# facebookresearch/NeRF-Det

Hardware: AMD Instinct MI355X
Metric: scenes/sec (50-view 240x320, 40x40x16 voxels) (higher is better)
Workload: dtype f32 (convolutions: fp32 operands as hi + lo fp16 pairs of the power-of-two pre-scaled tensors, three products per multiply on the fp16 MFMA, fp32 accumulate; error against fp64 at or below the six-product bf16x3 form's; a device-side range guard repeats a scene on bf16x3 when part of a tensor falls ; 1 GPU; cfg2: nerfdet_res50_2x_low_res forward_test, 50 views 240x320, 40x40x16 voxels, fp32, 1 scene/step/GPU, random-init weights; parallelism=scene replicas x1 (no data-path collective)

## Files before the change

include/nerfdet_hip.h:

```cpp
#ifndef NERFDET_HIP_H
#define NERFDET_HIP_H

#include <stdint.h>

#ifdef __cplusplus
extern "C" {
#endif

#define NDET_OK 0
#define NDET_E_INVALID (-1)
#define NDET_E_UNSUPPORTED (-2)
#define NDET_E_LAUNCH (-3)

#define NDET_LAYOUT_CN 0
#define NDET_LAYOUT_NC 1

int ndet_version(void);
const char* ndet_last_error(void);

int ndet_get_points(float* points, int nx, int ny, int nz, const float* voxel_size_host,
                    const float* origin_host, void* stream);

int ndet_nchw_to_nhwc(const float* src, float* dst, int n, int c, int hw, void* stream);

// ... 264 lines not shown
                      const float* residual, int relu, int splits, int tile, void* workspace, void* stream);

int ndet_conv_ndhwc(const float* in, const float* w_packed, float* out, int D, int H, int W, int Cin, int Cout,
                    const int* kernel_host, const int* stride_host, const int* pad_host, const float* scale,
                    const float* shift, const float* residual, int residual_up2, int relu, int splits, int tile,
                    void* workspace, void* stream);

int ndet_split_weights_bf16x3(const float* w_packed, int taps, int Cout, int Cin, uint16_t* planes, void* stream);

int ndet_split_weights_bf16x3_torch(const float* w_torch, int taps, int Cout, int Cin, int adjoint, uint16_t* planes, void* stream);

int ndet_point_mlp_alpha(const float* points, const float* global_feat, int N, int F, int K0, int hidden, const uint16_t* const* w_planes_host,
                         const float* w_inv_scale_host, const float* const* bias_host, const float* w_sigma, const float* b_sigma,
                         float* raw_sigma, float* alpha, float* h_out, void* stream);

int ndet_split_weights_f16x2(const float* w_packed, int taps, int Cout, int Cin, float scale, uint16_t* planes, void* stream);

int ndet_amax_f32(const float* x, int64_t n, float* slot, void* stream);

int ndet_amax_slot_floats(void);

int ndet_measurement_knob(const char* name_host, int64_t value);

typedef struct NdetConvArgs {
    int32_t size;
    const float* in;
    const uint16_t* w_planes;
    float* out;
    int D, H, W, Cin, Cout;
    int kernel[3], stride[3], pad[3];
    int transposed;
    const float* scale;
    const float* shift;
    const float* residual;
    int residual_up2, relu, splits, tile, arith;
    const float* in_amax;
    float w_inv_scale;
    const float* w_amax;
    float* out_amax;
    void* workspace;
    unsigned* guard;
    float guard_l1, guard_tol;
    int keep_partials;
    const float* map_w;
    const float* map_b;
    float* map_out;
} NdetConvArgs;
int ndet_conv_split(const NdetConvArgs* a, void* stream);

int ndet_conv_split_batch(const NdetConvArgs* a, int batch, void* stream);

int ndet_conv_halo_patch(int tile, int D, int H, int W, const int* kernel, int* patch, int* looped);

#define NDET_TILE_DIRECT 1
#define NDET_TILE_OWNS_ROWS 2
#define NDET_TILE_ORDER2 4
int ndet_conv_tile_info(int tile, int* rows, int* cols, int* flags);

int ndet_conv_chain(const float* in, const uint16_t* w_planes, int D, int H, int W, int Cin, int Cmid, const int* kernel,
                    const int* stride, const int* pad, const float* scale1, const float* shift1, const uint16_t* w3_planes,
                    int Cout, const float* scale3, const float* shift3, const float* residual, int relu3, float* out,
                    int arith, const float* in_amax, float w1_inv_scale, float w3_inv_scale, float* out_amax, float guard_l1,
                    float guard_l1_3, float guard_tol, unsigned* guard, void* stream);

int ndet_bottleneck_f16x2(const float* x, int N, int H, int W, int Cin, int Cout, const uint16_t* w1_planes, float w1_inv_scale, const float* scale1,
                          const float* shift1, const uint16_t* w2_planes, float w2_inv_scale, const float* scale2, const float* shift2,
                          const uint16_t* w3_planes, float w3_inv_scale, const float* scale3, const float* shift3, const uint16_t* wd_planes,
                          float wd_inv_scale, const float* scale_d, const float* shift_d, const float* in_amax, float* out_amax, float* out,
                          const float* guard_l1_host, float guard_tol, unsigned* guard, void* stream);

int ndet_bn_relu_maxpool_nhwc(const float* x, const float* scale, const float* shift, int N, int H, int W, int C,
                              float* out, void* stream);

int ndet_stem_pack_weights(const float* w_64x3x7x7, uint16_t* planes , void* stream);
int ndet_stem_pack_weights_f16x2(const float* w_64x3x7x7, float scale, uint16_t* planes , void* stream);

int ndet_stem_conv_bn_relu_maxpool(const float* images, int N, int H, int W, int64_t stride_n, int64_t stride_c, int64_t stride_y,
                                   int64_t stride_x, const uint16_t* w_planes, float w_inv_scale, const float* scale, const float* shift, float* out, float* out_amax,
                                   void* stream);

int ndet_normalize_views(const uint8_t* frames_bgr, const int* ids, int n_sel, int H, int W, const double* mean_rgb,
                         const double* std_rgb, float* img, float* denorm, void* stream);

int ndet_target_rays(const uint8_t* frames_bgr, const int* target_ids, int n_targets, int H, int W, int margin,
                     const float* intrinsic_rows, const float* camrotc2w, const float* cam_lightpos, const double* mean_rgb,
                     const double* std_rgb, float* raydirs, float* lightpos, float* gt_images, void* stream);

int ndet_resize_normalize_views(const uint8_t* frames_bgr, const int* ids, int n_sel, int Hs, int Ws, int Hr, int Wr, int H, int W,
                                const double* mean_rgb, const double* std_rgb, float* img, float* denorm, uint8_t* resized_bgr,
                                void* stream);

int ndet_resize_normalize_views_nv12(const uint8_t* surfaces, const int* ids, int n_sel, int Hs, int Ws, int pitch, int uv_row, int rows,
                                     int Hr, int Wr, int H, int W, const double* mean_rgb, const double* std_rgb, float* img, float* denorm,
                                     uint8_t* resized_bgr, void* stream);

int ndet_nv12_to_bgr(const uint8_t* surfaces, const int* ids, int n_sel, int Hs, int Ws, int pitch, int uv_row, int rows,
                     uint8_t* frames_bgr, void* stream);

int ndet_bgr_to_nv12(const uint8_t* frames_bgr, int n, int H, int W, uint8_t* surfaces, void* stream);

int ndet_depth_frames(const uint16_t* frames_mm, const int* ids, int n_sel, int Hd, int Wd, int h, int w, int margin, double* out,
                      void* stream);

int ndet_positive_indices(const double* x, int64_t n, int64_t* indices, int64_t* count, void* workspace, void* stream);

int ndet_camera_rays(const float* intrinsic_rows, const float* camrotc2w, const float* cam_lightpos, int n_cams, int x0, int y0, int stride,
// ... 84 lines not shown
```

nerf-det_amd/_lib.py:

```python
from __future__ import annotations

import ctypes
import os
from ctypes import c_char_p, c_float, c_int, c_int64, c_void_p

_HERE = os.path.dirname(os.path.abspath(__file__))
LIB_PATH = os.path.join(_HERE, "lib", "libnerfdet_hip.so")

NDET_LAYOUT_CN = 0
NDET_LAYOUT_NC = 1

_P = c_void_p
_F3 = ctypes.POINTER(c_float)


class NdetConvArgs(ctypes.Structure):
    _fields_ = ([("size", ctypes.c_int32), ("in_", _P), ("w_planes", _P), ("out", _P)] + [(f, c_int) for f in ("D", "H", "W", "Cin", "Cout")]
                + [(f, c_int * 3) for f in ("kernel", "stride", "pad")] + [("transposed", c_int), ("scale", _P), ("shift", _P), ("residual", _P)]
                + [(f, c_int) for f in ("residual_up2", "relu", "splits", "tile", "arith")] + [("in_amax", _P), ("w_inv_scale", c_float)]
                + [(f, _P) for f in ("w_amax", "out_amax", "workspace", "guard")] + [("guard_l1", c_float), ("guard_tol", c_float), ("keep_partials", c_int)]
                + [(f, _P) for f in ("map_w", "map_b", "map_out")])


class NdetDepthGate(ctypes.Structure):
# ... 74 lines not shown
                               _P, _P, _P, _G, _P], c_int),
    "ndet_scene_density_finish": ([_S, _P, _P, _P], c_int),
    "ndet_scene_volume_finish": ([_S, _P, _P, _P, _P], c_int),
    "ndet_scene_density_finish_ring": ([_S, c_int, _P, _P, _P], c_int),
    "ndet_scene_volume_finish_ring": ([_S, c_int, _P, _P, _P, _P], c_int),
    "ndet_scene_group_check": ([_SG, _GS, c_int], c_int),
    "ndet_scene_accumulate_group": ([_SG, _GS, c_int, _P, c_int, c_int, c_int64, c_int64, _P, c_int64, c_int64, _P, _P, c_int, c_int, c_int64, c_int64,
                                     c_int64, _P, _P, _G, _P], c_int),
    "ndet_scene_density_finish_group": ([_SG, _GS, _P, _P, _P], c_int),
    "ndet_scene_volume_finish_group": ([_SG, _GS, _P, _P, _P, _P], c_int),
    "ndet_scene_group_ring_check": ([_SG, _GR, _P], c_int),
    "ndet_scene_density_finish_group_ring": ([_SG, _GR, _P, _P, _P, _P, _P], c_int),
    "ndet_scene_volume_finish_group_ring": ([_SG, _GR, _P, _P, _P, _P, _P, _P], c_int),
    "ndet_alpha_gate": ([_P, _P, _P, _P, c_int, c_int, c_int, _P], c_int),
    "ndet_sigma_to_alpha": ([_P, _P, c_int, _P], c_int),
    "ndet_posenc_concat": ([_P, _P, c_int, c_int, c_int, _P, _P], c_int),
    "ndet_sigma_head": ([_P, c_int, _P, c_int, c_int, _P, _P, c_int, _P, _P, _P], c_int),
    "ndet_nms_workspace_bytes": ([c_int], c_int64),
    "ndet_aligned_3d_nms": ([_P, _P, _P, c_int, c_float, _P, _P, _P, _P], c_int),
    "ndet_head_decode": ([_P, c_int, _P, _P, c_int, c_int, c_int, _F3, _F3, _P, _P, _P, _P], c_int),
    "ndet_head_decode_levels": ([c_int, _P, _P, _P, _P, _P, _P, c_int, _P, c_int, c_int, c_int, _P, _P, _P, _P], c_int),
    "ndet_sample_along_rays": ([_P, _P, c_int, c_int, c_float, c_float, _P, _P, _P, _P], c_int),
    "ndet_ray_view_stats": ([_P, c_int, _P, c_int, c_float, c_float, _P, c_int, c_int, c_int64, c_int64, c_int64,
                             _P, c_int, c_int, c_int, c_int64, c_int64, _P, _P, _P, _P], c_int),
    "ndet_pack_rgb_nhwc4": ([_P, c_int, c_int, c_int, c_int64, c_int64, c_int64, _P, _P], c_int),
    "ndet_ray_view_stats_packed": ([_P, c_int, _P, c_int, c_float, c_float, _P, c_int, c_int, _P, c_int, c_int, c_int, c_int64, c_int64,
                                    _P, _P, _P, _P], c_int),
    "ndet_ray_view_stats_bank": ([_P, c_int, _P, c_int, c_float, c_float, c_int, c_int, c_int, c_int, c_int, _P, _P, _P, _P], c_int),
    "ndet_ray_view_stats_bank_group": ([_P, ctypes.POINTER(NdetBankGroupSel), c_float, c_float, c_int, c_int, c_int, c_int, c_int, _P, _P, _P, _P], c_int),
    "ndet_occupancy_bits": ([_P, _P, c_int, c_int, c_int, c_float, c_int, _P, _P], c_int),
    "ndet_cull_blocks": ([c_int64], c_int64),
    "ndet_cull_count": ([_P, c_int64, _P, ctypes.POINTER(c_int), _F3, _F3, c_int, _P, _P], c_int),
    "ndet_cull_write": ([_P, c_int64, _P, ctypes.POINTER(c_int), _F3, _F3, c_int, _P, _P, _P, _P], c_int),
    "ndet_ray_view_count_bank": ([_P, c_int64, _P, c_int, c_float, c_float, _P, _P, _P], c_int),
    "ndet_ray_advance": ([_P, _P, c_int, c_int, c_int, c_int, _P], c_int),
    "ndet_front_blocks": ([c_int64, c_int], c_int64),
    "ndet_front_count": ([_P, c_int, c_int, c_int, c_int, _P, c_float, _P, ctypes.POINTER(c_int), _F3, _F3, c_int, _P, _P], c_int),
    "ndet_front_write": ([_P, c_int, c_int, c_int, c_int, _P, c_float, _P, ctypes.POINTER(c_int), _F3, _F3, c_int, _P, _P, _P, _P], c_int),
    "ndet_ray_view_stats_packed_bwd": ([_P, _P, c_int, _P, c_int, c_float, c_float, _P, c_int, c_int, c_int, c_int64, c_int64, _P, _P], c_int),
    "ndet_project_sample": ([_P, c_int, _P, c_int, c_float, c_float, _P, c_int, c_int, c_int64, c_int64, c_int64,
                             _P, c_int, c_int, c_int, c_int64, c_int64, _P, _P, _P], c_int),
    "ndet_composite": ([_P, _P, _P, c_int, c_int, c_int, _P, _P, _P, _P, _P, _P, _P, _P], c_int),
    "ndet_sample_pdf": ([_P, _P, c_int, c_int, _P, c_int, c_int, _P, _P], c_int),
    "ndet_importance_merge": ([_P, _P, _P, _P, c_int, c_int, _P, c_int, c_int, _P, _P, _P, _P], c_int),
    "ndet_backproject_aggregate_bwd": ([_P, c_int, c_int, c_int, c_int, c_int, c_int64, c_int64, _P, c_int, _P, _P, _P], c_int),
    "ndet_density_features_bwd": ([_P, _P, c_int, c_int, c_int, c_int, c_int64, c_int64, _P, _P, c_int, _P, _P, _P, _P], c_int),
    "ndet_ray_view_stats_bwd": ([_P, _P, c_int, _P, c_int, c_float, c_float, _P, c_int, c_int, c_int, c_int64, c_int64, _P, _P], c_int),
    "ndet_composite_bwd": ([_P, _P, _P, c_int, c_int, c_int, _P, _P, _P, _P, _P], c_int),
    "ndet_split_weights_bf16x3": ([_P, c_int, c_int, c_int, _P, _P], c_int),
    "ndet_split_weights_f16x2": ([_P, c_int, c_int, c_int, c_float, _P, _P], c_int),
    "ndet_conv_split": ([ctypes.POINTER(NdetConvArgs), _P], c_int),
    "ndet_conv_split_batch": ([ctypes.POINTER(NdetConvArgs), c_int, _P], c_int),
    "ndet_conv_halo_patch": ([c_int] * 4 + [ctypes.POINTER(c_int)] * 3, c_int),
    "ndet_conv_tile_info": ([c_int] + [ctypes.POINTER(c_int)] * 3, c_int),
    "ndet_conv_chain": ([_P, _P] + [c_int] * 5 + [_P] * 6 + [c_int, _P, _P, _P, c_int, _P, c_int, _P, c_float, c_float, _P, c_float, c_float, c_float, _P, _P], c_int),
    "ndet_bottleneck_f16x2": ([_P, c_int, c_int, c_int, c_int, c_int, _P, c_float, _P, _P, _P, c_float, _P, _P, _P, c_float, _P, _P, _P, c_float, _P, _P, _P, _P, _P,
                               _P, c_float, _P, _P], c_int),
    "ndet_amax_f32": ([_P, ctypes.c_int64, _P, _P], c_int),
    "ndet_amax_slot_floats": ([], c_int),
    "ndet_point_mlp_alpha": ([_P, _P, c_int, c_int, c_int, c_int, _P, _P, _P, _P, _P, _P, _P, _P, _P], c_int),
    "ndet_measurement_knob": ([c_char_p, c_int64], c_int),
    "ndet_split_weights_bf16x3_torch": ([_P, c_int, c_int, c_int, c_int, _P, _P], c_int),
    "ndet_level_valid": ([_P, c_int, c_int, c_int, c_int, _P, _P], c_int),
    "ndet_select_candidates": ([c_int, _P, _P, _P, _P, c_float, _P, _P, _P, _P, _P], c_int),
    "ndet_select_candidates_topk": ([c_int, _P, _P, _P, _P, c_float, c_int, _P, _P, _P, _P, _P], c_int),
    "ndet_gather_detections": ([_P, c_int, _P, _P, _P, _P, _P, _P, _P], c_int),
    "ndet_nms_pack_detections": ([_P, _P, _P, _P, c_int, c_int, c_int, c_float, _P, _P, _P, _P, c_int, _P, _P], c_int),
    "ndet_normalize_views": ([_P, _P, c_int, c_int, c_int, _P, _P, _P, _P, _P], c_int),
    "ndet_target_rays": ([_P, _P, c_int, c_int, c_int, c_int, _P, _P, _P, _P, _P, _P, _P, _P, _P], c_int),
    "ndet_resize_normalize_views": ([_P, _P] + [c_int] * 7 + [_P] * 6, c_int),
    "ndet_resize_normalize_views_nv12": ([_P, _P] + [c_int] * 10 + [_P] * 6, c_int),
    "ndet_nv12_to_bgr": ([_P, _P] + [c_int] * 6 + [_P, _P], c_int),
    "ndet_bgr_to_nv12": ([_P] + [c_int] * 3 + [_P, _P], c_int),
    "ndet_depth_frames": ([_P, _P] + [c_int] * 6 + [_P, _P], c_int),
    "ndet_positive_indices": ([_P, c_int64, _P, _P, _P, _P], c_int),
    "ndet_positive_indices_workspace_bytes": ([c_int64], c_int64),
    "ndet_camera_rays": ([_P, _P, _P] + [c_int] * 6 + [_P, _P, _P], c_int),
    "ndet_pack_frames": ([_P, _P, _P, c_int64, _P, _P, _P], c_int),
    "ndet_frame_errors": ([_P, _P, _P, _P, c_int, c_int64, _P, _P], c_int),
    "ndet_frame_ssim": ([_P, _P, _P, c_int, c_int, c_int, c_int, _P, _P], c_int),
    "ndet_project_boxes": ([_P, _P, _P] + [c_int] * 7 + [c_float, _P, _P, _P, _P, _P], c_int),
    "ndet_draw_boxes": ([_P, _P, _P, _P] + [c_int] * 5 + [_P, _P], c_int),
    "ndet_label_frames": ([_P] * 5 + [c_int] * 7 + [_P, _P], c_int),
    "ndet_stem_pack_weights": ([_P, _P, _P], c_int),
    "ndet_stem_conv_bn_relu_maxpool": ([_P, c_int, c_int, c_int, c_int64, c_int64, c_int64, c_int64, _P, c_float, _P, _P, _P, _P, _P], c_int),
    "ndet_stem_pack_weights_f16x2": ([_P, c_float, _P, _P], c_int),
    "ndet_wgrad_dy_planes": ([_P, c_int, c_int, c_int, _P, _P], c_int),
    "ndet_wgrad_dy_planes_f16x2": ([_P, c_int, c_int, c_int, _P, _P, _P], c_int),
    "ndet_bn_workspace_floats": ([c_int64, c_int], c_int64),
    "ndet_bn_train_forward": ([_P, c_int64, c_int, _P, _P, _P, _P, c_float, c_float, _P, c_int, _P, _P, _P, _P, _P, _P], c_int),
    "ndet_bn_train_backward": ([_P, _P, _P, c_int64, c_int, _P, _P, _P, c_int, _P, _P, _P, _P, _P, _P, _P], c_int),
    "ndet_wgrad_to_torch": ([_P, c_int, c_int, c_int, c_int, _P, _P], c_int),
    "ndet_split_weights_train": ([_P, c_int, c_int, c_int, c_int, _P, _P, _P, _P], c_int),
    "ndet_relu_affine_bwd": ([_P, _P, _P, c_int64, c_int, c_int, _P, _P, _P], c_int),
    "ndet_relu_affine_bwd_amax": ([_P, _P, _P, c_int64, c_int, c_int, _P, _P, _P, _P], c_int),
    "ndet_wgrad_split": ([_P] + [c_int] * 4 + [_P, _P, _P, _P] + [c_int] * 4 + [_P, _P, _P, _P, c_int, _P], c_int),
    "ndet_wgrad_rows": ([_P] + [c_int] * 4 + [_P, _P, _P] + [c_int] * 3 + [_P, _P], c_int),
    "ndet_bn_relu_maxpool_nhwc": ([_P, _P, _P, c_int, c_int, c_int, c_int, _P, _P], c_int),
    "ndet_conv3d_workspace_bytes": ([c_int] * 8, c_int64),
    "ndet_conv_ndhwc": ([_P, _P, _P, c_int, c_int, c_int, c_int, c_int, ctypes.POINTER(c_int), ctypes.POINTER(c_int),
                         ctypes.POINTER(c_int), _P, _P, _P, c_int, c_int, c_int, c_int, _P, _P], c_int),
    "ndet_conv3d_ndhwc": ([_P, _P, _P, c_int, c_int, c_int, c_int, c_int, c_int, c_int, c_int, _P, _P, _P, c_int, c_int, c_int,
                           _P, _P], c_int),
}

_lib = None
# ... 58 lines not shown
```

nerf-det_amd/csrc/conv_split_kernels.hip:

```cpp
#include "conv_common.hpp"

#include "spl_common.hpp"

#include <type_traits>

template <int BM, int BN, int WGM, int WGN, int SCH, bool BATCH = false>
__device__ __forceinline__ void conv_split_mainloop(const Conv3dParams& p, const uint16_t* __restrict__ wsplit, uint16_t* lds16,
                                                    f32x16 (&acc)[BM / WGM / 32][BN / WGN / 32], int& ztap) {
    constexpr int NTHR = 64 * WGM * WGN;
    constexpr int WM = BM / WGM, WN = BN / WGN;
    constexpr int MT = WM / 32, NT = WN / 32;
    constexpr int RPA = NTHR / 8;
    constexpr int RPB = NTHR / 4;
    constexpr int AR = BM / RPA, BR = BN / RPB;
    static_assert(AR >= 1 && BR >= 1 && MT >= 1 && NT >= 1, "tile too small for the thread count");
    constexpr int APL = BM * SPL_RS, BPL = BN * SPL_RS;
    constexpr int NPL = Spl<SCH>::NPL, WPL = Spl<SCH>::WPL;
    const float xs = SCH == 1 ? conv_xscale(p.amax_in) : 1.0f;
    uint16_t* As = lds16;
    uint16_t* Bs = lds16 + NPL * APL;

    const int tid = threadIdx.x;
    const int lane = tid & 63, wave = tid >> 6;
    const int wm = wave / WGN, wn = wave % WGN;
// ... 1188 lines not shown
    NDET_REQUIRE(taps <= 32, NDET_E_UNSUPPORTED, "%s: the persistent 128x256 tile supports at most 32 taps", fn);
    NDET_REQUIRE(p.Cout % 16 == 0, NDET_E_UNSUPPORTED, "%s: the persistent 128x256 tile needs Cout %% 16 == 0", fn);
    NDET_REQUIRE((int64_t)p.D * p.H * p.W * p.Cin * 4 < ((int64_t)1 << 31) && (int64_t)taps * p.Cin * p.Cout * 6 < ((int64_t)1 << 31) &&
                     ((int64_t)p.M + 128) * p.Cout * 4 < ((int64_t)1 << 31),
                 NDET_E_UNSUPPORTED, "%s: the persistent 128x256 tile addresses at most 2 GB per operand", fn);
    const int n_mt = (p.M + BM - 1) / BM, n_nt = (p.Cout + WS_BN - 1) / WS_BN;
    const int64_t n_tiles = (int64_t)n_mt * n_nt * p.splits;
    static int n_cu = 0;
    if (n_cu == 0) {
        int dev = 0;
        hipDeviceProp_t prop;
        if (hipGetDevice(&dev) != hipSuccess || hipGetDeviceProperties(&prop, dev) != hipSuccess) n_cu = 256;
        else n_cu = prop.multiProcessorCount > 0 ? prop.multiProcessorCount : 256;
    }
    const int grid = (int)(n_tiles < n_cu ? n_tiles : n_cu);
    const int sch = conv_scheme(p);
    const size_t lds = (size_t)2 * (sch == 2 ? 1 : (sch == 1 ? 2 : 3)) * (BM + WS_BN) * CBK * sizeof(uint16_t);
    return with_scheme(sch, [&](auto s) -> int {
        const auto kernel = k_conv_split_wsp<decltype(s)::value, BM, NCONS>;
        NDET_RAISE_LDS(kernel, lds);
        hipLaunchKernelGGL(kernel, dim3(grid), dim3(64 * (NCONS + 4)), lds, st, p, (const uint16_t*)p.w, n_mt, n_nt);
        return NDET_OK;
    });
}


struct HaloGeom {
    int ltd, lth, ltw;
    int npd, nph, npw;
    int HH, HW, NH;
    int T;
    int KDL;
    int Tin;
};

struct HaloRowMap {
    int first, ltw, lth, d0, h0, w0, OD, OH, OW;
    __device__ __forceinline__ int operator()(int row) const {
        const int r = first + row;
        const int tw = r & ((1 << ltw) - 1), th = (r >> ltw) & ((1 << lth) - 1), td = r >> (ltw + lth);
        const int od = d0 + td, oh = h0 + th, ow = w0 + tw;
        return (od < OD && oh < OH && ow < OW) ? (od * OH + oh) * OW + ow : -1;
    }
};
struct HaloRowMapBatch {
    HaloRowMap in_volume;
    int vol_first;
    __device__ __forceinline__ int operator()(int row) const {
        const int m = in_volume(row);
        return m < 0 ? m : vol_first + m;
    }
};

template <int NT16, int WGN, int SCHB, int NPROD = 4>
__global__ __launch_bounds__(64 * (2 * WGN + NPROD), 1) void k_conv_split_halo(const Conv3dParams p, const uint16_t* __restrict__ wsplit, const HaloGeom g) {
    constexpr int SCH = SCHB & 3;
    constexpr bool BATCH = (SCHB & SPL_BATCH) != 0;
    constexpr int BN = 16 * NT16 * WGN;
    constexpr int NCONS = 2 * WGN, NTHR = 64 * (NCONS + NPROD);
    constexpr int PT = 64 * NPROD;
    constexpr int HALO_MAX = (BN == 128) ? 400 : 224;
    constexpr int NSTAGE = (BN == 128) ? 3 : 2;
    constexpr int NPIECE = (HALO_MAX * 8 + PT - 1) / PT;
    constexpr int APL = HALO_MAX * CBK, BPL = BN * CBK;
    constexpr int NPL = SCH == 1 ? 2 : (SCH == 2 ? 1 : 3);
    constexpr int WPL = SCH == 1 ? 2 : 3;
    constexpr int BSTAGE = NPL * BPL;
    constexpr int BR = BN / (16 * NPROD);
    static_assert(BR >= 1 && BN % (16 * NPROD) == 0, "every producer wave stages 16 rows of each row group");
    constexpr int NB = NPL * BR;
    extern __shared__ __attribute__((aligned(16))) uint16_t lds16[];
    uint16_t* Bs = lds16 + NPL * APL;

    const int tid = threadIdx.x;
    const int lane = tid & 63;
    const int wave = __builtin_amdgcn_readfirstlane(tid >> 6);
    const bool consumer = wave < NCONS;
    const int wm = (wave % NCONS) / WGN, wn = (wave % NCONS) % WGN;
    const ConvBlock blk = conv_block(p);
    const int n0 = blk.y * BN;
    const int TH = 1 << g.lth, TW = 1 << g.ltw;
    int pb = blk.x;
    const int pwi = pb % g.npw; pb /= g.npw;
    const int phi = pb % g.nph;
    const int pdv = pb / g.nph;
    const int vol = BATCH ? pdv / g.npd : 0;
    const int pdi = BATCH ? pdv - vol * g.npd : pdv;
    const int d0 = pdi << g.ltd, h0 = phi << g.lth, w0 = pwi << g.ltw;
    const float amax_in = conv_amax_in(p);
    conv_guard_check(p, amax_in);

    const int nch_all = p.Cin / CBK;
    int cb = 0, ce = nch_all;
    if (p.splits > 1) {
        cb = (int)((int64_t)nch_all * blk.z / p.splits);
        ce = (int)((int64_t)nch_all * (blk.z + 1) / p.splits);
    }
    const int nch = ce - cb;
    const int T = g.T, Tin = g.Tin;
    const int S = nch * T;
    const int nphase = nch * g.KDL;

    f32x4v acc[4][NT16];
#pragma unroll
    for (int a = 0; a < 4; ++a)
#pragma unroll
        for (int b = 0; b < NT16; ++b) acc[a][b] = (f32x4v){0.f, 0.f, 0.f, 0.f};

    if (!consumer) {
        const int stid = tid - 64 * NCONS;
        const int pw4 = wave - NCONS;
        const float xs = SCH == 1 ? conv_xscale(p.amax_in) : 1.0f;
        const int64_t slice = (int64_t)p.H * p.W * p.Cin;
        const bool dloop = g.KDL > 1;
        const __amdgpu_buffer_rsrc_t ares = __builtin_amdgcn_make_buffer_rsrc((void*)(p.in - (dloop ? p.pd * slice : 0)), 0, WS_OOB, 0x00020000);
        const __amdgpu_buffer_rsrc_t bres = __builtin_amdgcn_make_buffer_rsrc((void*)wsplit, 0, WS_OOB, 0x00020000);
        unsigned avoff[NPIECE], adst[NPIECE], amask[NPIECE];
#pragma unroll
        for (int i = 0; i < NPIECE; ++i) {
            const int idx = stid + PT * i;
            const int row = idx >> 3, q = idx & 7;
            const int hw = row % g.HW, hh = (row / g.HW) % g.HH, hd = row / (g.HW * g.HH);
            const int vd = d0 + hd - (dloop ? 0 : p.pd), vh = h0 - p.ph + hh, vw = w0 - p.pw + hw;
            const bool ok = row < g.NH && (unsigned)vd < (unsigned)p.D && (unsigned)vh < (unsigned)p.H && (unsigned)vw < (unsigned)p.W;
            if constexpr (BATCH) avoff[i] = ok ? (unsigned)((((int64_t)(vol * p.D + vd) * p.H + vh) * p.W + vw) * p.Cin * 4 + q * 16) : WS_OOB;
            else avoff[i] = ok ? (unsigned)((((int64_t)vd * p.H + vh) * p.W + vw) * p.Cin * 4 + q * 16) : WS_OOB;
            unsigned msk = 0;
            if (dloop)
                for (int k = 0; k < g.KDL; ++k)
                    if ((unsigned)(vd + k - p.pd) >= (unsigned)p.D) msk |= 1u << k;
            amask[i] = msk;
            adst[i] = row < g.NH ? (unsigned)((row * CBK + (((q >> 1) ^ ws_swz(row)) * 8) + (q & 1) * 4) * 2) : ~0u;
        }
        unsigned bvoff[BR];
#pragma unroll
        for (int i = 0; i < BR; ++i) {
            const int row = (stid >> 2) + (PT / 4) * i, co = n0 + row;
            bvoff[i] = co < p.Cout ? (unsigned)((co * CBK + (((stid & 3) ^ ws_swz(row)) * 8)) * 2) : WS_OOB;
        }
        const unsigned wtile_b = (unsigned)p.Cout * CBK * 2;
        int dt = 0, dc = 0;
        auto dma_b = [&](int u) {
            const unsigned soff = __builtin_amdgcn_readfirstlane((unsigned)(((int64_t)dt * nch_all + cb + dc) * WPL) * wtile_b);
            uint16_t* stage = Bs + (u % NSTAGE) * BSTAGE;
#pragma unroll
            for (int i = 0; i < BR; ++i)
#pragma unroll
                for (int pl = 0; pl < NPL; ++pl) {
                    uint16_t* dst = stage + pl * BPL + ((PT / 4) * i + pw4 * 16) * CBK;
                    spl_dma16(bres, dst, bvoff[i], __builtin_amdgcn_readfirstlane(soff + pl * wtile_b));
                }
            if (++dt == T) { dt = 0; ++dc; }
        };
        u32x4 ra[NPIECE];
        auto load_a = [&](int a) {
            const int c = a / g.KDL, kdl = a - c * g.KDL;
            const unsigned soff = __builtin_amdgcn_readfirstlane((unsigned)(((cb + c) * CBK + (dloop ? kdl * slice : 0)) * 4));
            const unsigned sh = 31 - kdl;
#pragma unroll
            for (int i = 0; i < NPIECE; ++i) ra[i] = __builtin_amdgcn_raw_buffer_load_b128(ares, ((amask[i] << sh) & WS_OOB) | avoff[i], soff, 0);
        };
        auto split_store_a = [&]() {
            char* base = reinterpret_cast<char*>(lds16);
#pragma unroll
            for (int i = 0; i < NPIECE; ++i) {
                const u32x4 u = ra[i];
                uint2 s0, s1, s2;
                const float4 xv = make_float4(__uint_as_float(u.x), __uint_as_float(u.y), __uint_as_float(u.z), __uint_as_float(u.w));
                spl_split<SCH>(xv, xs, s0, s1, s2);
                if (adst[i] != ~0u) {
                    *reinterpret_cast<uint2*>(base + adst[i]) = s0;
                    if (NPL > 1) *reinterpret_cast<uint2*>(base + adst[i] + APL * 2) = s1;
                    if (NPL > 2) *reinterpret_cast<uint2*>(base + adst[i] + APL * 4) = s2;
                }
            }
        };

        __builtin_amdgcn_s_setprio(3);
        load_a(0);
#pragma unroll
        for (int u = 0; u < NSTAGE - 1; ++u)
            if (u < S) dma_b(u);
        split_store_a();
        if (nphase > 1) load_a(1);
        asm volatile("s_waitcnt vmcnt(0)" ::: "memory");
        __syncthreads();
        int s = 0;
        for (int ci = 0; ci < nphase; ++ci) {
            for (int t = 0; t < Tin; ++t, ++s) {
                if (s + NSTAGE - 1 < S) {
                    dma_b(s + NSTAGE - 1);
                    if (NSTAGE == 3) {
                        asm volatile("s_waitcnt vmcnt(%0)" ::"n"(NB) : "memory");
                    } else {
                        asm volatile("s_waitcnt vmcnt(0)" ::: "memory");
                    }
                } else {
                    asm volatile("s_waitcnt vmcnt(0)" ::: "memory");
                }
                __syncthreads();
            }
            if (ci + 1 < nphase) {
                split_store_a();
                __syncthreads();
                if (ci + 2 < nphase) load_a(ci + 2);
            }
        }
    } else {
        const int frow = lane & 15, fc = lane >> 4;
        int hr0[4];
#pragma unroll
        for (int ta = 0; ta < 4; ++ta) {
            const int r = wm * 64 + ta * 16 + frow;
            const int tw = r & (TW - 1), th = (r >> g.ltw) & (TH - 1), td = r >> (g.ltw + g.lth);
            hr0[ta] = (td * g.HH + th) * g.HW + tw;
        }
        const int boff = (wn * (16 * NT16) + frow) * CBK + ((fc ^ ws_swz(frow)) * 8);
        const int wkh = p.kh, wkw = p.kw;
        __syncthreads();
        int s = 0;
        for (int ci = 0; ci < nphase; ++ci) {
            int kd = 0, kh = 0, kw = 0;
            for (int t = 0; t < Tin; ++t, ++s) {
                const int tapoff = (kd * g.HH + kh) * g.HW + kw;
                const uint16_t* bst = Bs + (s % NSTAGE) * BSTAGE + boff;
                bf16x8 fa[NPL][4], fb[NPL][NT16];
                const uint16_t* ap[4];
#pragma unroll
                for (int ta = 0; ta < 4; ++ta) {
                    const int hr = hr0[ta] + tapoff;
                    ap[ta] = lds16 + hr * CBK + ((fc ^ ws_swz(hr)) * 8);
                }
#pragma unroll
                for (int pl = 0; pl < NPL; ++pl) {
                    const int pq = NPL - 1 - pl;
#pragma unroll
                    for (int ta = 0; ta < 4; ++ta) fa[pl][ta] = *reinterpret_cast<const bf16x8*>(ap[ta] + pl * APL);
#pragma unroll
                    for (int tb = 0; tb < NT16; ++tb) fb[pq][tb] = *reinterpret_cast<const bf16x8*>(bst + pq * BPL + tb * 16 * CBK);
                }
#pragma unroll
                for (int order = NPL - 1; order >= 0; --order)
                    if (order <= p.max_order)
#pragma unroll
                    for (int pa = 0; pa <= order; ++pa) {
                        const int pbb = order - pa;
#pragma unroll
                        for (int ta = 0; ta < 4; ++ta)
#pragma unroll
                            for (int tb = 0; tb < NT16; ++tb) {
                                acc[ta][tb] = spl_mfma16<SCH>(fa[pa][ta], fb[pbb][tb], acc[ta][tb]);
                            }
                    }
                if (++kw == wkw) {
                    kw = 0;
                    if (++kh == wkh) { kh = 0; ++kd; }
                }
                __syncthreads();
            }
            if (ci + 1 < nphase) __syncthreads();
        }
    }
    __builtin_amdgcn_s_setprio(0);

    constexpr int CLDC = BN + 4;
    float* Cs = reinterpret_cast<float*>(lds16);
    float mx = 0.0f;
    for (int h = 0; h < 2; ++h) {
        if (consumer && wm == h) {
#pragma unroll
            for (int ta = 0; ta < 4; ++ta)
#pragma unroll
                for (int tb = 0; tb < NT16; ++tb)
#pragma unroll
                    for (int r = 0; r < 4; ++r)
                        Cs[(ta * 16 + (lane >> 4) * 4 + r) * CLDC + wn * (16 * NT16) + tb * 16 + (lane & 15)] = acc[ta][tb][r];
        }
        __syncthreads();
        const HaloRowMap rmap{h * 64, g.ltw, g.lth, d0, h0, w0, p.OD, p.OH, p.OW};
        const float osc = conv_oscale_of(p, amax_in);
        float* Wl = Cs + 64 * CLDC;
        if (p.map_out && h == 0)
            for (int i = tid; i < BN * 8; i += NTHR) reinterpret_cast<float4*>(Wl)[i] = reinterpret_cast<const float4*>(p.map_w)[i];
        if constexpr (BATCH) conv_store_rows_mapped<BN, NTHR>(p, Cs, CLDC, 64, n0, tid, 0, blk.z, HaloRowMapBatch{rmap, vol * p.OD * p.OH * p.OW}, mx, osc);
        else conv_store_rows_mapped<BN, NTHR>(p, Cs, CLDC, 64, n0, tid, 0, blk.z, rmap, mx, osc);
        __syncthreads();
        if (p.map_out) conv_map_rows<BN, NTHR>(p, Cs, CLDC, tid, rmap, osc, Wl);
    }
    if (p.amax_out && conv_writes_final(p)) conv_amax_commit(p.amax_out, mx);
}

static bool halo_geometry(const Conv3dParams& p, int halo_max, HaloGeom& g) {
    double best = 1e30;
    for (int dloop = 0; dloop <= (p.kd > 1 ? 1 : 0); ++dloop)
        for (int ltd = 0; ltd <= 7; ++ltd)
            for (int lth = 0; lth + ltd <= 7; ++lth) {
                const int ltw = 7 - ltd - lth;
                const int TD = 1 << ltd, TH = 1 << lth, TW = 1 << ltw;
                const int HD = dloop ? TD : TD + p.kd - 1, HH = TH + p.kh - 1, HW = TW + p.kw - 1;
                const int NH = HD * HH * HW;
                if (NH > halo_max) continue;
                const int npd = (p.OD + TD - 1) / TD, nph = (p.OH + TH - 1) / TH, npw = (p.OW + TW - 1) / TW;
                const double waste = (double)npd * TD * nph * TH * npw * TW / ((double)p.OD * p.OH * p.OW);
                const int kdl = dloop ? p.kd : 1;
                const double cost = waste * (1.0 + 0.03 * NH * kdl / 128.0);
                if (cost < best) {
                    best = cost;
                    g.ltd = ltd; g.lth = lth; g.ltw = ltw; g.npd = npd; g.nph = nph; g.npw = npw; g.HH = HH; g.HW = HW; g.NH = NH;
                    g.KDL = kdl;
                }
            }
    g.T = p.kd * p.kh * p.kw;
    g.Tin = g.T / (best < 1e29 ? g.KDL : 1);
    return best < 1e29;
}

template <int NT16, int WGN, int SCH, int NPROD, bool BATCH>
static int split_launch_halo(const Conv3dParams& p, int batch, hipStream_t st, const char* fn) {
    constexpr int NPL = SCH == 1 ? 2 : (SCH == 2 ? 1 : 3);
    constexpr int BN = 16 * NT16 * WGN, HALO_MAX = (BN == 128) ? 400 : 224, NSTAGE = (BN == 128) ? 3 : 2;
    NDET_REQUIRE(!p.transposed && p.sd == 1 && p.sh == 1 && p.sw == 1 && (p.kd & 1) && (p.kh & 1) && (p.kw & 1) && p.pd == p.kd / 2 &&
                     p.ph == p.kh / 2 && p.pw == p.kw / 2,
                 NDET_E_UNSUPPORTED, "%s: the halo tile needs a stride-1 same-padded convolution with odd kernel extents", fn);
    const int64_t nvol = BATCH ? batch : 1;
    NDET_REQUIRE(nvol * p.D * p.H * p.W * p.Cin * 4 < ((int64_t)1 << 31) && (int64_t)p.kd * p.kh * p.kw * p.Cin * p.Cout * 6 < ((int64_t)1 << 31),
                 NDET_E_UNSUPPORTED, "%s: the halo tile addresses at most 2 GB per operand", fn);
    NDET_REQUIRE(p.splits <= p.Cin / CBK, NDET_E_INVALID, "%s: the halo tile splits K over the %d channel chunks only", fn, p.Cin / CBK);
    HaloGeom g;
    NDET_REQUIRE(halo_geometry(p, HALO_MAX, g), NDET_E_UNSUPPORTED, "%s: no patch shape fits the halo tile", fn);
    dim3 grid((unsigned)(nvol * g.npd * g.nph * g.npw), (p.Cout + BN - 1) / BN, p.splits);
    size_t lds = (size_t)(NPL * HALO_MAX * CBK + NSTAGE * NPL * BN * CBK) * sizeof(uint16_t);
    const size_t cs = (size_t)64 * (BN + 4) * sizeof(float);
    if (cs > lds) lds = cs;
    const size_t lds_map = cs + (size_t)BN * 32 * sizeof(float);
    const size_t lds_cap = lds_map > lds ? lds_map : lds;
    if (p.map_out) {
        NDET_REQUIRE(p.Cout == BN && p.splits == 1 && !p.res && p.relu == 0, NDET_E_UNSUPPORTED,
                     "%s: the chained projection needs a tile that owns all %d output channels of its rows, no split-K / residual / ReLU", fn, p.Cout);
        lds = lds_cap;
    }
    const auto kernel = k_conv_split_halo<NT16, WGN, SCH + (BATCH ? SPL_BATCH : 0), NPROD>;
    NDET_RAISE_LDS(kernel, lds_cap);
    hipLaunchKernelGGL(kernel, grid, dim3(64 * (2 * WGN + NPROD)), lds, st, p, (const uint16_t*)p.w, g);
    return NDET_OK;
}

template <int BM, int BN, int WGM, int WGN, int SCH, bool BATCH>
static int split_launch_tile_sch(const Conv3dParams& p, hipStream_t st, const char* fn) {
    const int zdim = p.transposed ? 8 : p.splits;
    dim3 grid((p.M + BM - 1) / BM, (p.Cout + BN - 1) / BN, zdim);
    size_t lds = (size_t)Spl<SCH>::NPL * (BM + BN) * SPL_RS * sizeof(uint16_t);
    const size_t cs = (size_t)(BM / WGM) * (BN + 4) * sizeof(float);
    if (cs > lds) lds = cs;
    const auto kernel = k_conv_split<BM, BN, WGM, WGN, SCH + (BATCH ? SPL_BATCH : 0)>;
    if (lds > 64 * 1024) NDET_RAISE_LDS(kernel, lds);
    hipLaunchKernelGGL(kernel, grid, dim3(64 * WGM * WGN), lds, st, p, (const uint16_t*)p.w);
    return NDET_OK;
}
template <int BM, int BN, int WGM, int WGN>
static int split_launch_tile(const Conv3dParams& p, hipStream_t st, const char* fn) {
    return with_scheme(conv_scheme(p), [&](auto s) { return split_launch_tile_sch<BM, BN, WGM, WGN, decltype(s)::value, false>(p, st, fn); });
}
template <int BM, int BN, int WGM, int WGN>
static int split_launch_tile_batch(const Conv3dParams& p, int, hipStream_t st, const char* fn) {
    return with_scheme(conv_scheme(p), [&](auto s) { return split_launch_tile_sch<BM, BN, WGM, WGN, decltype(s)::value, true>(p, st, fn); });
}
template <int NT16, int WGN>
static int split_launch_halo_any(const Conv3dParams& p, hipStream_t st, const char* fn) {
    return with_scheme(conv_scheme(p), [&](auto s) { return split_launch_halo<NT16, WGN, decltype(s)::value, 4, false>(p, 1, st, fn); });
}
template <int NT16, int WGN>
static int split_launch_halo_any_batch(const Conv3dParams& p, int batch, hipStream_t st, const char* fn) {
    return with_scheme(conv_scheme(p), [&](auto s) { return split_launch_halo<NT16, WGN, decltype(s)::value, 4, true>(p, batch, st, fn); });
}
static int split_launch_halo_p8(const Conv3dParams& p, hipStream_t st, const char* fn) {
    return with_scheme(conv_scheme(p), [&](auto s) {
        constexpr int SCH = decltype(s)::value;
        return split_launch_halo<4, 4, SCH, SCH == 0 ? 4 : 8, false>(p, 1, st, fn);
    });
}
static int split_launch_halo_p8_batch(const Conv3dParams& p, int batch, hipStream_t st, const char* fn) {
    return with_scheme(conv_scheme(p), [&](auto s) {
        constexpr int SCH = decltype(s)::value;
        return split_launch_halo<4, 4, SCH, SCH == 0 ? 4 : 8, true>(p, batch, st, fn);
    });
}

#ifndef NDET_ORDER_DEFAULT
#define NDET_ORDER_DEFAULT -1
#endif
static int64_t g_nt_bytes = (int64_t)32 << 20;
static bool g_order2 = true;
// ... 12 lines not shown
    ndet_set_error("%s: unknown knob '%s' (nt_bytes, order2, deterministic_scatter, wgrad_wide, wgrad_xcd)", fn, name);
    return NDET_E_INVALID;
}
extern "C" int ndet_amax_slot_floats(void) { return NDET_AMAX_SUB * NDET_AMAX_STRIDE; }

struct ConvTile {
    int id, rows, cols, flags;
    int (*launch)(const Conv3dParams&, hipStream_t, const char*);
    int (*launch_batch)(const Conv3dParams&, int batch, hipStream_t, const char*);
};
static const ConvTile CONV_TILES[] = {
    {64, 64, 64, NDET_TILE_ORDER2, split_launch_tile<64, 64, 2, 2>, split_launch_tile_batch<64, 64, 2, 2>},
    {128, 128, 128, NDET_TILE_ORDER2, split_launch_tile<128, 128, 2, 2>, split_launch_tile_batch<128, 128, 2, 2>},
    {12864, 128, 64, NDET_TILE_ORDER2, split_launch_tile<128, 64, 2, 2>, split_launch_tile_batch<128, 64, 2, 2>},
    {100064, 64, 64, NDET_TILE_ORDER2 | NDET_TILE_DIRECT, split_launch_tile<64, 64, 2, 2>, split_launch_tile_batch<64, 64, 2, 2>},
    {100128, 128, 128, NDET_TILE_ORDER2 | NDET_TILE_DIRECT, split_launch_tile<128, 128, 2, 2>, split_launch_tile_batch<128, 128, 2, 2>},
    {112864, 128, 64, NDET_TILE_ORDER2 | NDET_TILE_DIRECT, split_launch_tile<128, 64, 2, 2>, split_launch_tile_batch<128, 64, 2, 2>},
    {128256, 128, 256, NDET_TILE_ORDER2, split_launch_ws, split_launch_ws_batch},
    {129256, 128, 256, 0, split_launch_wsp<128, 4>, nullptr},
    {129257, 128, 256, 0, split_launch_wsp<128, 8>, nullptr},
    {129064, 64, 256, 0, split_launch_wsp<64, 4>, nullptr},
    {3128, 128, 128, 0, split_launch_halo_any<4, 2>, split_launch_halo_any_batch<4, 2>},
    {3256, 128, 256, NDET_TILE_OWNS_ROWS, split_launch_halo_any<8, 2>, split_launch_halo_any_batch<8, 2>},
    {3257, 128, 256, NDET_TILE_OWNS_ROWS, split_launch_halo_any<4, 4>, split_launch_halo_any_batch<4, 4>},
    {3258, 128, 256, NDET_TILE_OWNS_ROWS, split_launch_halo_p8, split_launch_halo_p8_batch},
};
static const ConvTile* conv_tile(int id) {
    for (const ConvTile& t : CONV_TILES)
        if (t.id == id) return &t;
    return nullptr;
}

extern "C" int ndet_conv_tile_info(int tile, int* rows, int* cols, int* flags) {
    const char* fn = "ndet_conv_tile_info";
    NDET_REQUIRE(rows && cols && flags, NDET_E_INVALID, "%s: null pointer", fn);
    const ConvTile* t = conv_tile(tile);
    NDET_REQUIRE(t, NDET_E_INVALID, "%s: unknown tile %d", fn, tile);
    *rows = t->rows; *cols = t->cols; *flags = t->flags;
    return NDET_OK;
}

extern "C" int ndet_conv_halo_patch(int tile, int D, int H, int W, const int* kernel, int* patch, int* looped) {
    const char* fn = "ndet_conv_halo_patch";
    NDET_REQUIRE(kernel && patch && looped, NDET_E_INVALID, "%s: null pointer", fn);
    const ConvTile* t = conv_tile(tile);
    NDET_REQUIRE(t && (tile == 3128 || (t->flags & NDET_TILE_OWNS_ROWS)), NDET_E_INVALID, "%s: tile %d is not a halo tile", fn, tile);
    NDET_REQUIRE(D > 0 && H > 0 && W > 0 && kernel[0] >= 1 && kernel[1] >= 1 && kernel[2] >= 1, NDET_E_INVALID, "%s: sizes must be positive", fn);
    Conv3dParams p{};
    p.OD = D; p.OH = H; p.OW = W; p.kd = kernel[0]; p.kh = kernel[1]; p.kw = kernel[2];
    HaloGeom g;
    NDET_REQUIRE(halo_geometry(p, t->cols == 128 ? 400 : 224, g), NDET_E_UNSUPPORTED, "%s: no patch shape fits the halo tile", fn);
    patch[0] = 1 << g.ltd; patch[1] = 1 << g.lth; patch[2] = 1 << g.ltw;
    *looped = g.KDL > 1 ? 1 : 0;
    return NDET_OK;
}

static int conv_split_launch_n(Conv3dParams& p, int tile, bool keep_partials, int batch, hipStream_t st, const char* fn) {
    p.nt = (p.splits <= 1 || p.transposed) && (int64_t)p.M * p.Cout * 4 * (p.transposed ? 8 : 1) >= conv_nt_bytes() ? 1 : 0;
    const int64_t big_tiles = (int64_t)((p.M + 127) / 128) * ((p.Cout + 127) / 128);
    if (tile == 0) tile = (big_tiles >= 192 && p.Cout >= 128) ? 128 : 64;
    const ConvTile* t = conv_tile(tile);
    NDET_REQUIRE(t, NDET_E_INVALID, "%s: unknown tile %d", fn, tile);
    NDET_REQUIRE(batch == 1 || t->launch_batch, NDET_E_UNSUPPORTED, "%s: tile %d takes one volume per launch", fn, tile);
    p.direct = (t->flags & NDET_TILE_DIRECT) ? 1 : 0;
    NDET_REQUIRE(!p.direct || (!p.transposed && p.splits == 1 && p.Cout % 32 == 0 && ((int64_t)p.M + 128) * p.Cout * 4 < ((int64_t)1 << 32)),
                 NDET_E_UNSUPPORTED, "%s: the direct epilogue needs splits == 1, no transposition, Cout %% 32 == 0 and an output below 4 GB", fn);
    {
        const int tm = t->rows, tn = t->cols;
        const int64_t mt = (p.M + tm - 1) / tm, nt = (p.Cout + tn - 1) / tn;
        const int64_t taps = p.transposed ? 1 : (int64_t)p.kd * p.kh * p.kw;
        const int64_t w_bytes = taps * p.Cin * p.Cout * 6, a_bytes = (int64_t)p.M * p.Cin * 4 * (p.sd * p.sh * p.sw);
        const int64_t save_w = (mt - 1) * w_bytes, save_a = (nt - 1) * a_bytes;
        p.order = NDET_ORDER_DEFAULT;
        if (NDET_ORDER_DEFAULT < 0) {
            p.order = 0;
            if (!p.transposed && mt > 1 && nt * p.splits > 1 && save_w > save_a && w_bytes > (8 << 20)) p.order = 1;
            if (g_order2 && p.order == 0 && !p.transposed && nt > 1 && mt >= 16 && w_bytes <= (2 << 20) && save_a >= (8 << 20) &&
                (t->flags & NDET_TILE_ORDER2)) p.order = 2;
        }
    }
    const int rc = batch == 1 ? t->launch(p, st, fn) : t->launch_batch(p, batch, st, fn);
    if (rc != NDET_OK) return rc;
    NDET_CHECK_LAUNCH(fn);
    if (keep_partials && p.splits > 1) return NDET_OK;
    return conv_splitk_reduce_launch(p, st, fn);
}
int conv_split_launch(Conv3dParams& p, int tile, bool keep_partials, hipStream_t st, const char* fn) {
    return conv_split_launch_n(p, tile, keep_partials, 1, st, fn);
}

__global__ __launch_bounds__(256) void k_split_weights(const float* __restrict__ w, int taps, int Cout, int Cin, uint16_t* __restrict__ out) {
    const int64_t i = ((int64_t)blockIdx.x * blockDim.x + threadIdx.x) * 2;
    const int64_t n = (int64_t)taps * Cout * Cin;
    if (i >= n) return;
    const int ci = (int)(i % Cin), co = (int)((i / Cin) % Cout), tap = (int)(i / ((int64_t)Cin * Cout));
    const float a = w[i], b = w[i + 1];
    const uint32_t o0 = spl_pack(a, b);
    const float ra = a - spl_lo(o0), rb = b - spl_hi(o0);
    const uint32_t o1 = spl_pack(ra, rb);
    const uint32_t o2 = spl_pack(ra - spl_lo(o1), rb - spl_hi(o1));
    const uint32_t o[3] = {o0, o1, o2};
    const int steps = Cin / CBK;
    uint16_t* dst = out + (((int64_t)tap * steps + ci / CBK) * 3 * Cout + co) * CBK + (ci % CBK);
#pragma unroll
    for (int pl = 0; pl < 3; ++pl) *reinterpret_cast<uint32_t*>(dst + (int64_t)pl * Cout * CBK) = o[pl];
}
// ... 404 lines not shown
```

Before: 146.4 scenes/s.

## Stage three weight taps per barrier interval in the 128-column halo conv

Adds a variant of the halo convolution kernel that loads three kernel taps of weights per synchronization interval into a double-buffered stage pair, instead of one tap per interval with a three-deep ring. Consumers software-pipeline fragment reads for the next tap while issuing MFMAs for the current one. The aim is fewer __syncthreads and producer waits per tap. The cost is more LDS for weight stages and more register pressure from doubled fragment buffers. It is selected automatically for the 128-column tile in the two- and one-plane schemes when the tap count is divisible by three, and it comes with optional timing-stamp instrumentation plus an API to force the old path.

```diff
diff --git a/include/nerfdet_hip.h b/include/nerfdet_hip.h
--- a/include/nerfdet_hip.h
+++ b/include/nerfdet_hip.h
@@ -340,6 +340,8 @@
 
 int ndet_conv_halo_patch(int tile, int D, int H, int W, const int* kernel, int* patch, int* looped);
 
+int ndet_conv_halo_taps(int mode, int tile, int arith, int taps_per_image, int* taps, int* lds_bytes);
+
 #define NDET_TILE_DIRECT 1
 #define NDET_TILE_OWNS_ROWS 2
 #define NDET_TILE_ORDER2 4
diff --git a/nerf-det_amd/_lib.py b/nerf-det_amd/_lib.py
--- a/nerf-det_amd/_lib.py
+++ b/nerf-det_amd/_lib.py
@@ -150,6 +150,7 @@
     "ndet_conv_split": ([ctypes.POINTER(NdetConvArgs), _P], c_int),
     "ndet_conv_split_batch": ([ctypes.POINTER(NdetConvArgs), c_int, _P], c_int),
     "ndet_conv_halo_patch": ([c_int] * 4 + [ctypes.POINTER(c_int)] * 3, c_int),
+    "ndet_conv_halo_taps": ([c_int] * 4 + [ctypes.POINTER(c_int)] * 2, c_int),
     "ndet_conv_tile_info": ([c_int] + [ctypes.POINTER(c_int)] * 3, c_int),
     "ndet_conv_chain": ([_P, _P] + [c_int] * 5 + [_P] * 6 + [c_int, _P, _P, _P, c_int, _P, c_int, _P, c_float, c_float, _P, c_float, c_float, c_float, _P, _P], c_int),
     "ndet_bottleneck_f16x2": ([_P, c_int, c_int, c_int, c_int, c_int, _P, c_float, _P, _P, _P, c_float, _P, _P, _P, c_float, _P, _P, _P, c_float, _P, _P, _P, _P, _P,
diff --git a/nerf-det_amd/csrc/conv_split_kernels.hip b/nerf-det_amd/csrc/conv_split_kernels.hip
--- a/nerf-det_amd/csrc/conv_split_kernels.hip
+++ b/nerf-det_amd/csrc/conv_split_kernels.hip
@@ -1264,15 +1264,31 @@
     }
 };
 
+#define SPL_TPS3 8
+#ifdef HALO_STAMPS
+__device__ unsigned long long* g_halo_stamps = nullptr;
+extern "C" int ndet_halo_set_stamps(unsigned long long* buf) { return hipMemcpyToSymbol(HIP_SYMBOL(g_halo_stamps), &buf, sizeof(buf)) == hipSuccess ? 0 : -3; }
+#define HSTAMP_BEGIN() unsigned long long hs_acc[4] = {0, 0, 0, 0}, hs_t = __builtin_amdgcn_s_memtime()
+#define HSTAMP(i) do { __builtin_amdgcn_sched_barrier(0); const unsigned long long hs_n = __builtin_amdgcn_s_memtime(); hs_acc[i] += hs_n - hs_t; hs_t = hs_n; __builtin_amdgcn_sched_barrier(0); } while (0)
+#define HSTAMP_READS() do { if (HALO_STAMPS > 1) { asm volatile("s_waitcnt lgkmcnt(0)" ::: "memory"); HSTAMP(0); } } while (0)
+#define HSTAMP_END() do { if (g_halo_stamps && blockIdx.x == 0 && blockIdx.y == 0 && blockIdx.z == 0 && lane == 0) for (int i = 0; i < 4; ++i) g_halo_stamps[wave * 4 + i] = hs_acc[i]; } while (0)
+#else
+#define HSTAMP_BEGIN()
+#define HSTAMP(i)
+#define HSTAMP_READS()
+#define HSTAMP_END()
+#endif
 template <int NT16, int WGN, int SCHB, int NPROD = 4>
 __global__ __launch_bounds__(64 * (2 * WGN + NPROD), 1) void k_conv_split_halo(const Conv3dParams p, const uint16_t* __restrict__ wsplit, const HaloGeom g) {
     constexpr int SCH = SCHB & 3;
     constexpr bool BATCH = (SCHB & SPL_BATCH) != 0;
+    constexpr int TPS = (SCHB & SPL_TPS3) ? 3 : 1;
     constexpr int BN = 16 * NT16 * WGN;
     constexpr int NCONS = 2 * WGN, NTHR = 64 * (NCONS + NPROD);
     constexpr int PT = 64 * NPROD;
     constexpr int HALO_MAX = (BN == 128) ? 400 : 224;
-    constexpr int NSTAGE = (BN == 128) ? 3 : 2;
+    constexpr int NSTAGE = (BN == 128 && TPS == 1) ? 3 : 2;
+    static_assert(TPS == 1 || (BN == 128 && SCH != 0), "three taps per interval: the 128-column tile in the two- and one-plane schemes");
     constexpr int NPIECE = (HALO_MAX * 8 + PT - 1) / PT;
     constexpr int APL = HALO_MAX * CBK, BPL = BN * CBK;
     constexpr int NPL = SCH == 1 ? 2 : (SCH == 2 ? 1 : 3);
@@ -1281,6 +1297,7 @@
     constexpr int BR = BN / (16 * NPROD);
     static_assert(BR >= 1 && BN % (16 * NPROD) == 0, "every producer wave stages 16 rows of each row group");
     constexpr int NB = NPL * BR;
+    static_assert((size_t)(NPL * APL + NSTAGE * TPS * BSTAGE) * sizeof(uint16_t) <= 160 * 1024, "image + weight stages exceed a CU's LDS");
     extern __shared__ __attribute__((aligned(16))) uint16_t lds16[];
     uint16_t* Bs = lds16 + NPL * APL;
 
@@ -1354,7 +1371,7 @@
         int dt = 0, dc = 0;
         auto dma_b = [&](int u) {
             const unsigned soff = __builtin_amdgcn_readfirstlane((unsigned)(((int64_t)dt * nch_all + cb + dc) * WPL) * wtile_b);
-            uint16_t* stage = Bs + (u % NSTAGE) * BSTAGE;
+            uint16_t* stage = Bs + (TPS == 1 ? u % NSTAGE : u) * BSTAGE;
 #pragma unroll
             for (int i = 0; i < BR; ++i)
 #pragma unroll
@@ -1390,34 +1407,58 @@
 
         __builtin_amdgcn_s_setprio(3);
         load_a(0);
-#pragma unroll
-        for (int u = 0; u < NSTAGE - 1; ++u)
-            if (u < S) dma_b(u);
+        if constexpr (TPS == 1) {
+#pragma unroll
+            for (int u = 0; u < NSTAGE - 1; ++u)
+                if (u < S) dma_b(u);
+        } else {
+#pragma unroll
+            for (int j = 0; j < TPS; ++j) dma_b(j);
+        }
         split_store_a();
         if (nphase > 1) load_a(1);
         asm volatile("s_waitcnt vmcnt(0)" ::: "memory");
         __syncthreads();
+        HSTAMP_BEGIN();
         int s = 0;
         for (int ci = 0; ci < nphase; ++ci) {
-            for (int t = 0; t < Tin; ++t, ++s) {
-                if (s + NSTAGE - 1 < S) {
-                    dma_b(s + NSTAGE - 1);
-                    if (NSTAGE == 3) {
-                        asm volatile("s_waitcnt vmcnt(%0)" ::"n"(NB) : "memory");
+            if constexpr (TPS == 1) {
+                for (int t = 0; t < Tin; ++t, ++s) {
+                    if (s + NSTAGE - 1 < S) {
+                        dma_b(s + NSTAGE - 1);
+                        if (NSTAGE == 3) {
+                            asm volatile("s_waitcnt vmcnt(%0)" ::"n"(NB) : "memory");
+                        } else {
+                            asm volatile("s_waitcnt vmcnt(0)" ::: "memory");
+                        }
                     } else {
                         asm volatile("s_waitcnt vmcnt(0)" ::: "memory");
                     }
-                } else {
+                    HSTAMP(0);
+                    __syncthreads();
+                    HSTAMP(1);
+                }
+            } else {
+                for (int t = 0; t < Tin; t += TPS, ++s) {
+                    if ((s + 1) * TPS < S) {
+#pragma unroll
+                        for (int j = 0; j < TPS; ++j) dma_b(((s + 1) & 1) * TPS + j);
+                    }
                     asm volatile("s_waitcnt vmcnt(0)" ::: "memory");
-                }
-                __syncthreads();
+                    HSTAMP(0);
+                    __syncthreads();
+                    HSTAMP(1);
+                }
             }
             if (ci + 1 < nphase) {
                 split_store_a();
+                HSTAMP(2);
                 __syncthreads();
                 if (ci + 2 < nphase) load_a(ci + 2);
-            }
-        }
+                HSTAMP(3);
+            }
+        }
+        HSTAMP_END();
     } else {
         const int frow = lane & 15, fc = lane >> 4;
         int hr0[4];
@@ -1430,9 +1471,11 @@
         const int boff = (wn * (16 * NT16) + frow) * CBK + ((fc ^ ws_swz(frow)) * 8);
         const int wkh = p.kh, wkw = p.kw;
         __syncthreads();
+        HSTAMP_BEGIN();
         int s = 0;
         for (int ci = 0; ci < nphase; ++ci) {
             int kd = 0, kh = 0, kw = 0;
+            if constexpr (TPS == 1) {
             for (int t = 0; t < Tin; ++t, ++s) {
                 const int tapoff = (kd * g.HH + kh) * g.HW + kw;
                 const uint16_t* bst = Bs + (s % NSTAGE) * BSTAGE + boff;
@@ -1451,6 +1494,7 @@
 #pragma unroll
                     for (int tb = 0; tb < NT16; ++tb) fb[pq][tb] = *reinterpret_cast<const bf16x8*>(bst + pq * BPL + tb * 16 * CBK);
                 }
+                HSTAMP_READS();
 #pragma unroll
                 for (int order = NPL - 1; order >= 0; --order)
                     if (order <= p.max_order)
@@ -1468,10 +1512,65 @@
                     kw = 0;
                     if (++kh == wkh) { kh = 0; ++kd; }
                 }
+                HSTAMP(1);
                 __syncthreads();
-            }
-            if (ci + 1 < nphase) __syncthreads();
-        }
+                HSTAMP(2);
+            }
+            } else {
+                const uint16_t* ap[4];
+                auto read_frags = [&](bf16x8 (&fa)[NPL][4], bf16x8 (&fb)[NPL][NT16], const uint16_t* bst) {
+                    const int tapoff = (kd * g.HH + kh) * g.HW + kw;
+#pragma unroll
+                    for (int ta = 0; ta < 4; ++ta) {
+                        const int hr = hr0[ta] + tapoff;
+                        ap[ta] = lds16 + hr * CBK + ((fc ^ ws_swz(hr)) * 8);
+                    }
+#pragma unroll
+                    for (int pl = 0; pl < NPL; ++pl) {
+                        const int pq = NPL - 1 - pl;
+#pragma unroll
+                        for (int ta = 0; ta < 4; ++ta) fa[pl][ta] = *reinterpret_cast<const bf16x8*>(ap[ta] + pl * APL);
+#pragma unroll
+                        for (int tb = 0; tb < NT16; ++tb) fb[pq][tb] = *reinterpret_cast<const bf16x8*>(bst + pq * BPL + tb * 16 * CBK);
+                    }
+                    if (++kw == wkw) {
+                        kw = 0;
+                        if (++kh == wkh) { kh = 0; ++kd; }
+                    }
+                };
+                for (int t = 0; t < Tin; t += TPS, ++s) {
+                    const uint16_t* bst = Bs + (s & 1) * (TPS * BSTAGE) + boff;
+                    bf16x8 fa[2][NPL][4], fb[2][NPL][NT16];
+                    read_frags(fa[0], fb[0], bst);
+                    HSTAMP_READS();
+#pragma unroll
+                    for (int tt = 0; tt < TPS; ++tt) {
+                        if (tt + 1 < TPS) read_frags(fa[(tt + 1) & 1], fb[(tt + 1) & 1], bst + (tt + 1) * BSTAGE);
+#pragma unroll
+                        for (int order = NPL - 1; order >= 0; --order)
+                            if (order <= p.max_order)
+#pragma unroll
+                            for (int pa = 0; pa <= order; ++pa) {
+                                const int pbb = order - pa;
+#pragma unroll
+                                for (int ta = 0; ta < 4; ++ta)
+#pragma unroll
+                                    for (int tb = 0; tb < NT16; ++tb) {
+                                        acc[ta][tb] = spl_mfma16<SCH>(fa[tt & 1][pa][ta], fb[tt & 1][pbb][tb], acc[ta][tb]);
+                                    }
+                            }
+                    }
+                    HSTAMP(1);
+                    __syncthreads();
+                    HSTAMP(2);
+                }
+            }
+            if (ci + 1 < nphase) {
+                __syncthreads();
+                HSTAMP(3);
+            }
+        }
+        HSTAMP_END();
     }
     __builtin_amdgcn_s_setprio(0);
 
@@ -1527,10 +1626,18 @@
     return best < 1e29;
 }
 
+static bool g_halo_tps1 = false;
+static constexpr bool halo_has_tps3(int cols, int sch, int nprod) { return cols == 128 && nprod == 4 && (sch == 1 || sch == 2); }
+static int halo_tps(int cols, int sch, int nprod, int tin) { return halo_has_tps3(cols, sch, nprod) && tin % 3 == 0 && !g_halo_tps1 ? 3 : 1; }
+static constexpr size_t halo_walk_lds(int cols, int sch, int tps) {
+    const int npl = sch == 1 ? 2 : (sch == 2 ? 1 : 3);
+    const int halo_max = cols == 128 ? 400 : 224, nstage = (cols == 128 && tps == 1) ? 3 : 2;
+    return (size_t)(npl * halo_max * CBK + nstage * tps * npl * cols * CBK) * sizeof(uint16_t);
+}
+
 template <int NT16, int WGN, int SCH, int NPROD, bool BATCH>
 static int split_launch_halo(const Conv3dParams& p, int batch, hipStream_t st, const char* fn) {
-    constexpr int NPL = SCH == 1 ? 2 : (SCH == 2 ? 1 : 3);
-    constexpr int BN = 16 * NT16 * WGN, HALO_MAX = (BN == 128) ? 400 : 224, NSTAGE = (BN == 128) ? 3 : 2;
+    constexpr int BN = 16 * NT16 * WGN, HALO_MAX = (BN == 128) ? 400 : 224;
     NDET_REQUIRE(!p.transposed && p.sd == 1 && p.sh == 1 && p.sw == 1 && (p.kd & 1) && (p.kh & 1) && (p.kw & 1) && p.pd == p.kd / 2 &&
                      p.ph == p.kh / 2 && p.pw == p.kw / 2,
                  NDET_E_UNSUPPORTED, "%s: the halo tile needs a stride-1 same-padded convolution with odd kernel extents", fn);
@@ -1541,7 +1648,8 @@
     HaloGeom g;
     NDET_REQUIRE(halo_geometry(p, HALO_MAX, g), NDET_E_UNSUPPORTED, "%s: no patch shape fits the halo tile", fn);
     dim3 grid((unsigned)(nvol * g.npd * g.nph * g.npw), (p.Cout + BN - 1) / BN, p.splits);
-    size_t lds = (size_t)(NPL * HALO_MAX * CBK + NSTAGE * NPL * BN * CBK) * sizeof(uint16_t);
+    const int tps = halo_tps(BN, SCH, NPROD, g.Tin);
+    size_t lds = halo_walk_lds(BN, SCH, tps);
     const size_t cs = (size_t)64 * (BN + 4) * sizeof(float);
     if (cs > lds) lds = cs;
     const size_t lds_map = cs + (size_t)BN * 32 * sizeof(float);
@@ -1550,6 +1658,15 @@
         NDET_REQUIRE(p.Cout == BN && p.splits == 1 && !p.res && p.relu == 0, NDET_E_UNSUPPORTED,
                      "%s: the chained projection needs a tile that owns all %d output channels of its rows, no split-K / residual / ReLU", fn, p.Cout);
         lds = lds_cap;
+    }
+    if constexpr (halo_has_tps3(BN, SCH, NPROD)) {
+        static_assert(halo_walk_lds(BN, SCH, 3) <= 160 * 1024, "image + two three-tap weight stages exceed a CU's LDS");
+        if (tps == 3) {
+            const auto kernel3 = k_conv_split_halo<NT16, WGN, SCH + (BATCH ? SPL_BATCH : 0) + SPL_TPS3, NPROD>;
+            NDET_RAISE_LDS(kernel3, lds_cap);
+            hipLaunchKernelGGL(kernel3, grid, dim3(64 * (2 * WGN + NPROD)), lds, st, p, (const uint16_t*)p.w, g);
+            return NDET_OK;
+        }
     }
     const auto kernel = k_conv_split_halo<NT16, WGN, SCH + (BATCH ? SPL_BATCH : 0), NPROD>;
     NDET_RAISE_LDS(kernel, lds_cap);
@@ -1668,6 +1785,24 @@
     NDET_REQUIRE(halo_geometry(p, t->cols == 128 ? 400 : 224, g), NDET_E_UNSUPPORTED, "%s: no patch shape fits the halo tile", fn);
     patch[0] = 1 << g.ltd; patch[1] = 1 << g.lth; patch[2] = 1 << g.ltw;
     *looped = g.KDL > 1 ? 1 : 0;
+    return NDET_OK;
+}
+
+extern "C" int ndet_conv_halo_taps(int mode, int tile, int arith, int taps_per_image, int* taps, int* lds_bytes) {
+    const char* fn = "ndet_conv_halo_taps";
+    NDET_REQUIRE(mode >= -1 && mode <= 1, NDET_E_INVALID, "%s: mode is -1 (leave), 0 (automatic) or 1 (one tap per interval)", fn);
+    if (taps || lds_bytes) {
+        const ConvTile* t = conv_tile(tile);
+        NDET_REQUIRE(t && (tile == 3128 || (t->flags & NDET_TILE_OWNS_ROWS)), NDET_E_INVALID, "%s: tile %d is not a halo tile", fn, tile);
+        NDET_REQUIRE(arith >= 0 && arith <= 2 && taps_per_image >= 1, NDET_E_INVALID, "%s: arith is 0 / 1 / 2, taps_per_image >= 1", fn);
+    }
+    if (mode >= 0) g_halo_tps1 = mode == 1;
+    if (taps || lds_bytes) {
+        const int nprod = tile == 3258 && arith != 0 ? 8 : 4;
+        const int tps = halo_tps(conv_tile(tile)->cols, arith, nprod, taps_per_image);
+        if (taps) *taps = tps;
+        if (lds_bytes) *lds_bytes = (int)halo_walk_lds(conv_tile(tile)->cols, arith, tps);
+    }
     return NDET_OK;
 }
 
```

New measurement: 147.9 scenes/s, median of 6. 1.1% higher.
